# Funatiq/cuclark

Measured on AMD Instinct MI355X. Metric: Mreads/sec (10M x 150bp, k=31), higher is better.
Workload: dtype u64

## Files before the change

cuclark_amd/_lib.py:

```python
import ctypes as C
import importlib.util
import os
import subprocess

_PKG = os.path.dirname(os.path.abspath(__file__))
LIB_PATH = os.environ.get("MIC_LIB_PATH") or os.path.join(_PKG, "lib", "libmi_clark.so")
CSRC = os.path.join(_PKG, "csrc")

MIC_RESULT_WORDS = 8
MIC_FLAG_ROW_OVERFLOW = 1
MIC_FLAG_DENSE_PATH = 2
MIC_ROW_INVALID = 0xFFFFFFFF
MIC_ROLLUP_WORDS, MIC_ROLLUP_MAX_LEVELS = 8, 7
MIC_ROLLUP_UNRESOLVED, MIC_ROLLUP_PENDING = 0xFFFFFFFF, 0xFFFFFFFE
MIC_DENSITY_WORDS, MIC_DENSITY_CONF_BINS, MIC_DENSITY_GAMMA_BINS = 5153, 51, 101
MIC_KSKETCH_REGS = 16384
MIC_LAYOUT_AUTO, MIC_LAYOUT_DIRECT, MIC_LAYOUT_MINIMIZER, MIC_LAYOUT_SUPER, MIC_LAYOUT_SUPER2 = 0, 1, 2, 3, 4


class MicError(RuntimeError):
    def __init__(self, code, msg):
        super().__init__(f"libmi_clark error {code}: {msg}")
        self.code = code

# ... 44 lines not shown
    ("mic_db_load_host", C.c_int, [_VP, _VP, C.c_uint64, _VP, C.c_int, _VP, C.c_uint32, C.c_uint64, C.c_uint64]),
    ("mic_db_load_device", C.c_int, [_VP, _VP, C.c_uint64, _VP, C.c_int, _VP, C.c_uint32, C.c_uint64, C.c_uint64]),
    ("mic_db_set_part", C.c_int, [_VP, C.c_uint32, C.c_uint32]),
    ("mic_db_reserve_hbm", C.c_int, [_VP, C.c_uint64]),
    ("mic_peer_matrix", C.c_int, [C.POINTER(C.c_int), C.c_int]),
    ("mic_device_memory", C.c_int, [C.c_int, C.POINTER(C.c_uint64), C.POINTER(C.c_uint64)]),
    ("mic_db_load_files_multi", C.c_int, [C.POINTER(C.c_void_p), _SZ, C.c_char_p, C.c_int, C.c_uint32]),
    ("mic_db_kernel_name", C.c_int, [_VP, C.c_char_p, _SZ]),
    ("mic_db_get_info", C.c_int, [_VP, C.POINTER(MicDbInfo)]),
    ("mic_db_unload", C.c_int, [_VP]),
    ("mic_db_last_build_report", C.c_char_p, []),
    ("mic_batches_alloc", C.c_int, [_VP, _SZ, _SZ, _SZ, _U32P, C.c_int, C.POINTER(_VP), C.POINTER(_VP), C.POINTER(_VP),
                                    C.POINTER(_VP)]),
    ("mic_batch_ready", C.c_int, [_VP, _SZ, _SZ, _SZ]),
    ("mic_batch_query", C.c_int, [_VP, _SZ, C.c_int, C.c_int]),
    ("mic_batch_wait", C.c_int, [_VP, _SZ]),
    ("mic_batch_dense_counts", C.c_int, [_VP, _SZ, _SZ, _VP]),
    ("mic_batch_check", C.c_int, [_VP, _SZ, C.POINTER(C.c_int)]),
    ("mic_batch_merge_shards", C.c_int, [C.POINTER(C.c_void_p), _SZ, _SZ]),
    ("mic_batch_query_group", C.c_int, [C.POINTER(C.c_void_p), _SZ, _SZ, C.c_int]),
    ("mic_sync", C.c_int, [_VP]),
    ("mic_thread_bind_near_device", C.c_int, [_VP, C.c_int]),
    ("mic_batches_free", C.c_int, [_VP]),
    ("mic_query_device", C.c_int, [_VP, _VP, _VP, _SZ, _VP, _VP, _VP]),
    ("mic_resolve_flagged_device", C.c_int, [_VP, _VP, _VP, _VP, _VP, _VP, C.POINTER(_SZ)]),
    ("mic_merge_rows_device", C.c_int, [_VP, _VP, _VP, _VP, _SZ, _VP]),
    ("mic_result_from_rows_device", C.c_int, [_VP, _VP, _VP, _SZ, _VP]),
    ("mic_count_dense_device", C.c_int, [_VP, _VP, _VP, _VP, _SZ, _VP, _VP]),
    ("mic_result_from_dense_device", C.c_int, [_VP, _VP, _VP, _SZ, _VP, _VP, _VP]),
    ("mic_probe_stats_device", C.c_int, [_VP, _VP, _VP, _SZ, C.POINTER(C.c_uint64)]),
    ("mic_last_query_ms", C.c_int, [_VP, C.POINTER(C.c_float)]),
    ("mic_last_crowd_stats", C.c_int, [_VP, C.POINTER(C.c_uint32)]),
    ("mic_debug_fetch_crowd", C.c_int, [_VP, _VP, _SZ, C.POINTER(C.c_uint32)]),
    ("mic_debug_stream_pool", C.c_int, [C.POINTER(C.c_uint32)]),
    ("mic_ingest_alloc", C.c_int, [_VP, _SZ, _SZ, C.POINTER(C.c_char_p), C.c_uint32, C.c_int, C.POINTER(_VP)]),
    ("mic_ingest_classify", C.c_int, [_VP, _SZ, _SZ, C.c_int, C.POINTER(MicIngestResult)]),
    ("mic_ingest_classify_group", C.c_int, [C.POINTER(C.c_void_p), _SZ, _SZ, _SZ, _SZ, C.c_int, C.POINTER(MicIngestResult)]),
    ("mic_ingest_fetch_group_rows", C.c_int, [_VP, _SZ, _SZ, _VP, _SZ, C.POINTER(C.c_uint64), C.POINTER(C.c_uint32)]),
    ("mic_ingest_group_stats", C.c_int, [_VP, C.POINTER(C.c_double), _SZ]),
    ("mic_ingest_fetch_packed", C.c_int, [_VP, _SZ, _VP, _SZ, _VP, _SZ, C.POINTER(C.c_uint64), C.POINTER(C.c_uint64)]),
    ("mic_ingest_free", C.c_int, [_VP]),
    ("mic_ingest_set_min_quality", C.c_int, [_VP, C.c_uint32]),
    ("mic_fastq_mask_quality", C.c_int, [_VP, _SZ, C.c_uint32, _VP]),
    ("mic_ingest_set_low_complexity", C.c_int, [_VP, C.c_uint32]),
    ("mic_text_mask_low_complexity", C.c_int, [_VP, _SZ, C.c_uint32, _VP]),
    ("mic_gz_inflate_device", C.c_int, [_VP, _VP, _SZ, C.POINTER(_VP), C.POINTER(_SZ), C.POINTER(C.c_uint32)]),
    ("mic_gz_copy_text", C.c_int, [_VP, _VP, _SZ, _SZ, _VP]),
    ("mic_gz_free_text", C.c_int, [_VP, _VP]),
    ("mic_gz_reserve", C.c_int, [_VP, _SZ, C.c_uint32]),
    ("mic_gz_reserve_bytes", C.c_uint64, [_SZ, C.c_uint32]),
    ("mic_gz_release", C.c_int, [_VP]),
    ("mic_pairs_index_device", C.c_int, [_VP, _VP, _SZ, _VP, _SZ, C.POINTER(_VP), C.POINTER(C.c_uint64), C.POINTER(C.c_uint32)]),
    ("mic_pairs_offsets", C.c_int, [_VP, C.POINTER(C.POINTER(C.c_uint64)), C.POINTER(_SZ), C.POINTER(C.c_uint32)]),
    ("mic_pairs_merge_to_slot", C.c_int, [_VP, _VP, C.c_uint64, C.c_uint64, _SZ, C.POINTER(_SZ)]),
    ("mic_pairs_text", C.c_int, [_VP, _VP, C.c_uint64, C.c_uint64, _VP, _SZ, C.POINTER(_SZ)]),
    ("mic_pairs_free", C.c_int, [_VP, _VP]),
    ("mic_text_index_device", C.c_int, [_VP, _VP, _SZ, C.POINTER(_VP), C.POINTER(C.c_uint64), C.POINTER(C.c_uint32)]),
    ("mic_text_index_front_device", C.c_int, [_VP, _VP, _SZ, C.POINTER(_VP), C.POINTER(C.c_uint64), C.POINTER(C.c_uint64), C.POINTER(C.c_uint32)]),
    ("mic_gz_stream_open", C.c_int, [_VP, _VP, _SZ, C.c_uint32, C.POINTER(_VP), C.POINTER(_VP), C.POINTER(_SZ)]),
    ("mic_gz_stream_next", C.c_int, [_VP, C.POINTER(_SZ), C.POINTER(C.c_int)]),
    ("mic_gz_stream_close", C.c_int, [_VP, C.c_int]),
    ("mic_text_offsets", C.c_int, [_VP, C.POINTER(C.POINTER(C.c_uint64)), C.POINTER(_SZ), C.POINTER(C.c_uint32)]),
    ("mic_text_to_slot", C.c_int, [_VP, _VP, C.c_uint64, C.c_uint64, _SZ, C.POINTER(_SZ)]),
    ("mic_text_copy", C.c_int, [_VP, _VP, C.c_uint64, C.c_uint64, _VP, _SZ, C.POINTER(_SZ)]),
    ("mic_text_free", C.c_int, [_VP, _VP]),
    ("mic_text_format", C.c_int, [_VP]),
# ... 119 lines not shown
```

cuclark_amd/csrc/mic_engine.hip:

```cpp
#include "mi_clark.h"
#include "mic_internal.h"

#include <errno.h>
#include <stdarg.h>
#include <stdio.h>
#include <stdlib.h>
#include <string.h>
#include <time.h>

#include <sched.h>

#include <algorithm>
#include <mutex>
#include <string>
#include <atomic>
#include <thread>
#include <unistd.h>
#include <utility>
#include <vector>

static thread_local char g_err[512] = "";
thread_local uint64_t mic_build_reserved_hbm = 0;

namespace {
// ... 623 lines not shown
  if (e->d_flagged) hipFree(e->d_flagged);
  if (e->d_crowd) hipFree(e->d_crowd);
  if (e->abund.d_counts) hipFree(e->abund.d_counts);
  if (e->rollup.d_counts) hipFree(e->rollup.d_counts);
  if (e->density.d_counts) hipFree(e->density.d_counts);
  if (e->ksketch.d_regs) hipFree(e->ksketch.d_regs);
  if (e->rollup.d_block) hipFree(e->rollup.d_block);
  if (e->ev0) mic_event_put(e->ev0);
  if (e->ev1) mic_event_put(e->ev1);
  if (e->stream) mic_stream_put(e->stream);
  if (e->up_stream) mic_stream_put(e->up_stream);
  if (e->down_stream) mic_stream_put(e->down_stream);
  delete e;
  return MIC_OK;
}

int mic_db_unload(mic_engine* e) {
  if (!e) return mic_set_error(MIC_E_INVALID, "null engine");
  int rc = set_device(e);
  if (rc) return rc;
  hipDeviceSynchronize();
  if (e->slots) hipFree(e->slots);
  if (e->side) hipFree(e->side);
  if (e->d_sizes) hipFree(e->d_sizes);
  e->slots = nullptr; e->side = nullptr; e->d_sizes = nullptr; e->db_loaded = false;
  memset(&e->info, 0, sizeof(e->info));
  return MIC_OK;
}

int mic_db_get_info(const mic_engine* e, mic_db_info* info) {
  if (!e || !info) return mic_set_error(MIC_E_INVALID, "null argument");
  if (!e->db_loaded) return mic_set_error(MIC_E_STATE, "no database loaded");
  *info = e->info;
  return MIC_OK;
}

const char* mic_db_last_build_report(void) {
  static thread_local std::string copy;
  std::lock_guard<std::mutex> lk(g_report_mu);
  copy = g_report;
  return copy.c_str();
}

int mic_db_reserve_hbm(mic_engine* e, uint64_t bytes) {
  if (!e) return mic_set_error(MIC_E_INVALID, "null engine");
  e->reserve_hbm = bytes;
  return MIC_OK;
}

int mic_db_set_part(mic_engine* e, uint32_t part, uint32_t n_parts) {
  if (!e) return mic_set_error(MIC_E_INVALID, "null engine");
  if (n_parts > 1 && part >= n_parts) return mic_set_error(MIC_E_INVALID, "part %u of %u", part, n_parts);
  if (n_parts > 65536) return mic_set_error(MIC_E_INVALID, "too many parts");
  if (e->db_loaded) return mic_set_error(MIC_E_STATE, "set the part before the database is loaded");
  e->part = n_parts > 1 ? part : 0; e->n_parts = n_parts > 1 ? n_parts : 0;
  return MIC_OK;
}

int mic_db_load_device(mic_engine* e, const uint8_t* d_sizes, uint64_t htsize, const void* d_keys, int key_bytes,
                       const uint16_t* d_labels, uint32_t sampling, uint64_t s0, uint64_t s1) {
  if (!e || !d_sizes || !d_keys || !d_labels) return mic_set_error(MIC_E_INVALID, "null argument");
  if (key_bytes != 2 && key_bytes != 4 && key_bytes != 8) return mic_set_error(MIC_E_INVALID, "key_bytes must be 2, 4 or 8");
  int rc = set_device(e);
  if (rc) return rc;
  if ((rc = check_shard(htsize, s0, s1))) return rc;
  if ((rc = apply_part(e, htsize, s0, s1))) return rc;
// ... 726 lines not shown
```

cuclark_amd/csrc/mic_kernels.hip:

```cpp
#include "mic_internal.h"
#include "mic_device.h"
#include "mic_ksketch.h"
#include "mic_hitmap.h"
#include "mic_join2.h"

#include <stdlib.h>
#include <type_traits>

#ifndef MIC_EXP
#define MIC_EXP 0
#endif
#ifndef MIC_FUNNEL64
#define MIC_FUNNEL64 1
#endif
#ifndef MIC_X
#define MIC_X 0
#endif

namespace {

__device__ __forceinline__ uint4 load_slot_quarter(const uint4* p) {
  typedef unsigned int u4 __attribute__((ext_vector_type(4)));
  u4 t = __builtin_nontemporal_load((const u4*)p);
  return make_uint4(t.x, t.y, t.z, t.w);
}

__device__ __forceinline__ uint64_t kmer_from_dwords(uint32_t d0, uint32_t d1, uint32_t d2, int nt_in_dword, int k) {
  const int s = 2 * nt_in_dword;
  uint64_t a = ((uint64_t)d0 << 32) | d1;
#if MIC_FUNNEL64
  uint64_t x = (a << s) | ((uint64_t)d2 >> (32 - s));
#else
  uint64_t x = s ? ((a << s) | (uint64_t)(d2 >> (32 - s))) : a;
#endif
  return x >> (64 - 2 * k);
}


struct ReadAhead { uint32_t pp, pe, hdr, w; };

__device__ __forceinline__ void ahead_ptr(const MicQueryArgs& a, uint32_t r, ReadAhead& x) {
  if (r < a.n_reads) { x.pp = a.reads_ptr[r]; x.pe = a.reads_ptr[r + 1]; } else { x.pp = 0; x.pe = 0; }
}

__device__ __forceinline__ void ahead_window(const uint16_t* __restrict__ cont, uint32_t r, uint32_t n_reads, int lane,
                                             ReadAhead& x) {
  x.hdr = 0; x.w = 0;
  if (r < n_reads) {
    const uint32_t pp = __builtin_amdgcn_readfirstlane(x.pp);
// ... 135 lines not shown
  uint32_t vbl = acc.label1, vbc = acc.count;
  if (n_ent > 1) {
    bl = __builtin_amdgcn_readlane(acc.label1, 0); bc = __builtin_amdgcn_readlane(acc.count, 0);
    for (uint32_t i = 1; i < n_ent; ++i) {
      const uint32_t l1 = __builtin_amdgcn_readlane(acc.label1, i);
      const uint32_t c = __builtin_amdgcn_readlane(acc.count, i);
      const bool over_best = c > bc || (c == bc && l1 < bl);
      const bool over_second = c > sc || (c == sc && l1 < sl);
      if (over_best) { sc = bc; sl = bl; bc = c; bl = l1; }
      else if (over_second) { sc = c; sl = l1; }
    }
    vbl = bl; vbc = bc;
  }
  uint32_t flags = 0;
  if (a.rows) {
    uint32_t* row = a.rows + (size_t)r * a.row_words;
    bool fits = n_ent <= a.row_words - 1 && !overflow;
    uint32_t rank = 0;
    for (uint32_t i = 0; i < n_ent; ++i) {
      uint32_t li = __builtin_amdgcn_readlane(acc.label1, i);
      rank += li < acc.label1;
    }
    bool big = (uint32_t)lane < n_ent && acc.count > 0xFFFF;
    if (__ballot(big)) fits = false;
    if (fits) {
      if ((uint32_t)lane < n_ent) row[1 + rank] = (acc.count << 16) | (acc.label1 - 1);
      if (lane == 0) row[0] = n_ent;
    } else {
      if (lane == 0) row[0] = MIC_ROW_INVALID;
      flags |= MIC_FLAG_ROW_OVERFLOW_;
    }
  }
  if (overflow) flags |= MIC_FLAG_ROW_OVERFLOW_;
  if (lane == 0) {
    uint4 lo, hi;
    lo.x = total;
    lo.y = vbl;
    lo.z = vbc;
    lo.w = sl;
    hi.x = sc;
    hi.y = n_ent; hi.z = flags; hi.w = 0;
    uint4* out = (uint4*)(a.results + (size_t)r * 8);
    out[0] = lo; out[1] = hi;
  }
#if MIC_EXP & 2
  if (__builtin_expect(__builtin_amdgcn_readfirstlane(flags) != 0, 0)) if (a.flagged) {
#else
  if (__builtin_amdgcn_readfirstlane(flags) && a.flagged) {
#endif
    if (lane == 0) {
      uint32_t pos = atomicAdd(&a.flagged[0], 1u);
      if (pos < a.flagged_cap) a.flagged[1 + pos] = r;
    }
  }
}

template <bool KEY64>
__global__ void __launch_bounds__(256) query_kernel(const MicQueryArgs a) {
  const int lane = threadIdx.x & 63;
  const int j = lane & 3;
  const uint32_t wave0 = __builtin_amdgcn_readfirstlane(blockIdx.x * 4 + (threadIdx.x >> 6));
  const uint32_t n_waves = gridDim.x * 4;
  const MicTable& t = a.t;
  const int k = t.k;
  const uint4* __restrict__ slots = t.slots;
  const uint16_t* __restrict__ cont = a.cont;

// ... 729 lines not shown
              }
            }
          }
        };
        while (__ballot(sl0 != 0xFFFFFFFFu) | __ballot(sl1 != 0xFFFFFFFFu)) {
          uint32_t nx0, nx1;
          level(sl0, sl1, res0, res1, nx0, nx1);
          sl0 = nx0; sl1 = nx1;
        }
        tally2(res0, res1, acc, n_ent, overflow, total, lane);
      }
    }
    uint32_t t_hdr, t_pp, t_pe;
    asm volatile("s_waitcnt vmcnt(0)" ::: "memory");
    __builtin_amdgcn_wave_barrier();
    ahead_take(ahead_sel ? ahead1 : ahead0, n_pp, t_hdr, t_pp, t_pe);
    __builtin_amdgcn_wave_barrier();
    {
      uint64_t kp = (uint64_t)__builtin_amdgcn_kernarg_segment_ptr();
      asm volatile("" : "+s"(kp));
      const __attribute__((address_space(4))) MicQueryArgs* kc = (const __attribute__((address_space(4))) MicQueryArgs*)kp;
      struct { uint32_t* results; uint32_t* rows; uint32_t* flagged; uint32_t row_words, flagged_cap; } fa;
      fa.results = kc->results; fa.rows = kc->rows; fa.flagged = kc->flagged; fa.row_words = kc->row_words; fa.flagged_cap = kc->flagged_cap;
      finish_read(acc, n_ent, total, overflow, r, fa, lane);
    }
    ahead_issue(ahead_sel ? ahead0 : ahead1, t_pp, r + 3 * n_waves);
    ahead_sel ^= 1;
    cur_pp = n_pp; cur_pe = n_pe; cur_hdr = t_hdr; n_pp = t_pp; n_pe = t_pe;
  }
}


__device__ __forceinline__ uint64_t wballot(bool p) { return __builtin_amdgcn_ballot_w64(p); }

static_assert(MIC_RMAX <= 32, "tally_counts sums the first two rows of lanes");
#define MIC_R_CROWDED (-16)
__device__ __forceinline__ void tally_counts(uint32_t lab1, uint32_t cnt, RowAcc& acc, uint32_t& n_ent, uint32_t& overflow,
                                             uint32_t& total, int lane) {
  uint64_t mm = wballot(lab1 != 0);
  while (mm) {
    const uint32_t l1 = __builtin_amdgcn_readlane(lab1, __builtin_ctzll(mm));
    const bool mine = lab1 == l1;
    mm &= ~wballot(mine);
    const uint32_t c = mine ? cnt : 0u;
    uint32_t sum = 0;
    {
      uint32_t v = c;
      v += (uint32_t)__builtin_amdgcn_update_dpp(0, (int)v, 0x111, 0xF, 0xF, true);
      v += (uint32_t)__builtin_amdgcn_update_dpp(0, (int)v, 0x112, 0xF, 0xF, true);
      v += (uint32_t)__builtin_amdgcn_update_dpp(0, (int)v, 0x114, 0xF, 0xF, true);
      v += (uint32_t)__builtin_amdgcn_update_dpp(0, (int)v, 0x118, 0xF, 0xF, true);
      sum = __builtin_amdgcn_readlane(v, 15) + __builtin_amdgcn_readlane(v, 31);
    }
    total += sum;
    row_add(acc, n_ent, overflow, l1, sum, lane);
  }
}

template <int KK, int MM, bool FWD, bool PART>
__global__ void __launch_bounds__(64 * MIC_M_WPB, 32 / MIC_M_WPB) query_kernel_r(const MicQueryArgs a) {
  __shared__ uint4 s_stage[MIC_M_WPB][MIC_RMAX * MIC_MSTRIDE + (MIC_RMAX / 8 - 1) * MIC_R_SKEW];
  __shared__ uint16_t s_rec[MIC_M_WPB][132];
  __shared__ uint32_t s_ahead[MIC_M_WPB][2][64];
  __shared__ uint32_t s_part[PART ? MIC_M_WPB : 1][2];
  const int lane = threadIdx.x & 63;
  const int wv = __builtin_amdgcn_readfirstlane(threadIdx.x >> 6);
  uint4* stage = s_stage[wv];
  uint16_t* rec = s_rec[wv];
  const uint32_t wave0 = __builtin_amdgcn_readfirstlane(blockIdx.x * MIC_M_WPB + wv);
  const uint32_t n_waves = gridDim.x * MIC_M_WPB;
  const MicTable& t = a.t;
  if (PART) { if (lane == 0) { s_part[wv][0] = t.slot_lo; s_part[wv][1] = t.slot_cnt; } __builtin_amdgcn_wave_barrier(); }
  const int k = KK ? KK : t.k, m = MM ? MM : t.m, ctx = k - m;
  const uint4* __restrict__ slots = t.slots;
  const uint16_t* __restrict__ cont = a.cont;
  auto below = [](uint64_t mask) { return (uint32_t)__builtin_amdgcn_mbcnt_hi((uint32_t)(mask >> 32), __builtin_amdgcn_mbcnt_lo((uint32_t)mask, 0u)); };

  uint32_t* ahead0 = s_ahead[wv][0];
  uint32_t* ahead1 = s_ahead[wv][1];
  auto ahead_issue = [&](uint32_t* entry, uint32_t pp_w, uint32_t r_ptr) {
    const uint64_t abase = ((uint64_t)(cont + pp_w)) & ~3ULL;
    const uint32_t rr = r_ptr < a.n_reads ? r_ptr : a.n_reads - 1;
    const uint64_t pbase = (uint64_t)(a.reads_ptr + rr) - 48;
    int ln = lane;
    asm volatile("" : "+v"(ln));
    if (ln < 12)
      __builtin_amdgcn_global_load_lds((const __attribute__((address_space(1))) void*)((const uint32_t*)abase + lane),
                                       (__attribute__((address_space(3))) void*)entry, 4, 0, 0);
    uint64_t pb = pbase + 48;
    asm volatile("" : "+s"(pb));
    if (ln < 2)
      __builtin_amdgcn_global_load_lds((const __attribute__((address_space(1))) void*)((const uint32_t*)pb + lane),
                                       (__attribute__((address_space(3))) void*)(entry + 12), 4, 0, 0);
  };
  auto ahead_take = [&](const uint32_t* entry, uint32_t pp_w, uint32_t& hdr, uint32_t& npp, uint32_t& npe) {
    const uint32_t raw = entry[lane];
    npp = __builtin_amdgcn_readlane(raw, 12); npe = __builtin_amdgcn_readlane(raw, 13);
    const bool odd = (((uint64_t)(cont + pp_w)) >> 1) & 1;
    const uint32_t first = __builtin_amdgcn_readfirstlane(raw);
    hdr = odd ? first >> 16 : first & 0xFFFFu;
  };
  auto ahead_word = [&](const uint32_t* entry, uint32_t pp_w) {
    const uint32_t raw = entry[lane];
    const bool odd = (((uint64_t)(cont + pp_w)) >> 1) & 1;
    const uint32_t up = (uint32_t)__builtin_amdgcn_update_dpp(0, (int)raw, 0x101, 0xF, 0xF, true);
    return __builtin_amdgcn_perm(up, raw, odd ? 0x05040706u : 0x03020504u);
  };
  uint32_t cur_pp, cur_pe, cur_hdr, n_pp, n_pe, ahead_sel;
  {
    const uint32_t r0 = wave0 < a.n_reads ? wave0 : a.n_reads - 1;
    cur_pp = __builtin_amdgcn_readfirstlane(a.reads_ptr[r0]); cur_pe = __builtin_amdgcn_readfirstlane(a.reads_ptr[r0 + 1]);
    ahead_issue(ahead0, cur_pp, wave0 + n_waves);
    asm volatile("s_waitcnt vmcnt(0)" ::: "memory");
    __builtin_amdgcn_wave_barrier();
    ahead_take(ahead0, cur_pp, cur_hdr, n_pp, n_pe);
    ahead_issue(ahead1, n_pp, wave0 + 2 * n_waves);
    ahead_sel = 1;
  }
  constexpr bool PIPE = KK != 0 && (MIC_R_PIPE >= 2 || (MIC_R_PIPE == 1 && FWD));
  struct Round {
    uint32_t G0, G1, G2, cur;
    int jmax, jmin, remaining;
  };
  struct NoGap {};
  struct Gap { uint32_t len1, b2, g0; };
  auto front = [&](const uint32_t first, const uint32_t cend, const uint32_t base, const uint32_t nk, const bool use_ahead, uint32_t& wd_out,
                   const auto gp) __attribute__((always_inline)) -> uint32_t {
    constexpr bool GAP = std::is_same<decltype(gp), const Gap>::value;
    int ln = lane;
    asm volatile("" : "+v"(ln));
    uint32_t wd;
    if constexpr (GAP) {
      const uint32_t* entry = ahead_sel ? ahead0 : ahead1;
      const uint32_t j = (uint32_t)ln < 12u ? (uint32_t)ln : 0u;
      const uint32_t d = j2_dword(j, gp.len1, gp.b2);
      wd = j2_window(ahead_word(entry, cur_pp), entry[d], entry[d + 1u], j, gp.len1, gp.b2);
    } else {
      wd = use_ahead ? ahead_word(ahead_sel ? ahead0 : ahead1, cur_pp)
                     : window_word_w(cont, first, cend, base, ln, false, 0u);
    }
    wd_out = wd;
    const uint32_t n_act = nk - base < 128u ? nk - base : 128u;
    if constexpr (KK == F3_K && MM == F3_M) {
      uint32_t p0, s0, s1, s2, q0, q1, q2;
      if constexpr (GAP) sampled_positions3<!FWD, true>(wd, lane, n_act, p0, s0, s1, s2, q0, q1, q2, gp.len1, gp.g0);
      else sampled_positions3<!FWD>(wd, lane, n_act, p0, s0, s1, s2, q0, q1, q2);
      const uint32_t pv = (uint32_t)__builtin_amdgcn_update_dpp(-1, (int)q2, 0x138, 0xF, 0xF, false);
      const bool f0 = q0 != pv, f1 = q1 != q0, f2 = q2 != q1;
      const uint64_t b0 = wballot(f0), b1 = wballot(f1), b2 = wballot(f2);
// ... 66 lines not shown
    region_x(G0, G1, key, xhi);
    bool rev = false;
    if (!FWD) {
      const uint32_t sh = 96u - 2u * (uint32_t)(k + ctx);
      const uint32_t r0 = __builtin_bitreverse32(G2), r1 = __builtin_bitreverse32(G1), r2 = __builtin_bitreverse32(G0);
      uint32_t q0, q1, q2;
      if (KK != 0 && sh != 0) {
        q0 = swap_comp_pairs(__builtin_amdgcn_alignbit(r0, r1, 33u - sh), __builtin_amdgcn_alignbit(r0, r1, 31u - sh));
        q1 = swap_comp_pairs(__builtin_amdgcn_alignbit(r1, r2, 33u - sh), __builtin_amdgcn_alignbit(r1, r2, 31u - sh));
        q2 = swap_comp_pairs(r2 << (sh - 1u), r2 << (sh + 1u));
      } else {
        q0 = sh ? __builtin_amdgcn_alignbit(r0, r1, 32u - sh) : r0;
        q1 = sh ? __builtin_amdgcn_alignbit(r1, r2, 32u - sh) : r1;
        q2 = r2 << sh;
        q0 = swap_comp_pairs(q0 >> 1, q0 << 1); q1 = swap_comp_pairs(q1 >> 1, q1 << 1); q2 = swap_comp_pairs(q2 >> 1, q2 << 1);
      }
      uint32_t kr, hr;
      region_x(q0, q1, kr, hr);
      rev = hr < xhi || (hr == xhi && kr < key);
      G0 = rev ? q0 : G0; G1 = rev ? q1 : G1; G2 = rev ? q2 : G2;
      key = rev ? kr : key; xhi = rev ? hr : xhi;
    }
    const int jmaxf = qa - i0, jminf = jmaxf - n + 1;
    const int jmax = rev ? ctx - jminf : jmaxf, jmin = rev ? ctx - jmaxf : jminf;
    uint32_t cur = vr ? sslot_of_x32(key, xhi, (uint32_t)t.n_main) : 0xFFFFFFFFu;
    bool mine = vr;
    if (PART) {
      mine = vr && cur - s_part[wv][0] < s_part[wv][1];
      cur = mine ? cur : 0xFFFFFFFFu;
    }
    L.G0 = G0; L.G1 = G1; L.G2 = G2; L.cur = cur;
    L.jmax = jmax; L.jmin = jmin; L.remaining = mine ? n : 0;
  };
  auto issue = [&](const uint32_t cur, const uint32_t nrun) __attribute__((always_inline)) {
    uint32_t sidx[MIC_RMAX / 8];
    int ln = lane;
    asm volatile("" : "+v"(ln));
    __builtin_amdgcn_wave_barrier();
    if (ln < MIC_RMAX) ((uint32_t*)stage)[lane] = cur;
    __builtin_amdgcn_wave_barrier();
    uint32_t so = (uint32_t)(uintptr_t)(__attribute__((address_space(3))) void*)stage;
    asm volatile("" : "+s"(so));
#pragma unroll
    for (int i = 0; i < MIC_RMAX / 8; ++i) sidx[i] = ((const uint32_t*)stage)[8 * i + (lane >> 3)];
#pragma unroll
    for (int i = 0; i < MIC_RMAX / 8; ++i) {
      if (8u * i >= nrun) break;
      if (sidx[i] != 0xFFFFFFFFu)
        __builtin_amdgcn_global_load_lds((const __attribute__((address_space(1))) void*)(slots + (uint64_t)sidx[i] * 8 + (lane & 7)),
                                         (__attribute__((address_space(3))) void*)(uintptr_t)(so + 16u * (64 + MIC_R_SKEW) * (uint32_t)i), 16, 0, 0);
    }
  };
  auto consume = [&](Round& L, RowAcc& acc, uint32_t& n_ent, uint32_t& overflow, uint32_t& total, uint32_t& cg) __attribute__((always_inline)) {
    const uint32_t G0 = L.G0, G1 = L.G1, G2 = L.G2;
    uint32_t key, xhi_;
    region_x(G0, G1, key, xhi_);
    const int jmax = L.jmax, jmin = L.jmin;
    uint32_t cur = L.cur;
    int remaining = L.remaining;
    bool again = false;
    do {
      if (again) issue(cur, MIC_RMAX);
      again = true;
      asm volatile("s_waitcnt vmcnt(0)" ::: "memory");
      __builtin_amdgcn_wave_barrier();
      const bool vl = cur != 0xFFFFFFFFu;
      const uint32_t* q = (const uint32_t*)(stage + (vl ? staged_at((uint32_t)lane) : 0));
      const uint4 ka = *(const uint4*)q;
      const uint2 kb = *(const uint2*)(q + 4);
      uint32_t e = (ka.x < key) + (ka.y < key) + (ka.z < key) + (ka.w < key) + (kb.x < key) + (kb.y < key);
      const uint32_t mz = q[30];
      bool more = vl && e < 6;
      e = e < 5 ? e : 5;
      for (;;) {
        uint32_t e3 = e + (e << 1);
        asm volatile("" : "+v"(e3));
        uint32_t g = q[e], S0 = q[6 + e3], S1 = q[7 + e3], S2 = q[8 + e3], pl = q[24 + e];
        asm volatile("" : "+v"(S2));
        const bool same = more && g == key;
        const uint32_t d0 = G0 ^ S0, d1 = G1 ^ S1, d2 = G2 ^ S2;
        const bool mineq = k > 16
                               ? ((d0 & ((1u << ((32 - 2 * ctx) & 31)) - 1u)) | (d1 >> xsh)) == 0
                               : (((((uint64_t)d0 << 32) | d1) << (2 * ctx)) >> (64 - 2 * m)) == 0;
        const uint32_t dl = d0 >> (32 - 2 * ctx);
        const uint32_t dr = k > 16 ? __builtin_amdgcn_alignbit(d1, d2, xsh)
                                        : (uint32_t)((((((uint64_t)d0 << 32) | d1)) << ((2 * k) & 63)) >> 32);
        const int left = __builtin_ctz(dl | (1u << (2 * ctx))) >> 1;
        const int right = __builtin_clz(dr | (1u << (31 - 2 * ctx))) >> 1;
        const int hi = left < jmax ? left : jmax, lo = ctx - right > jmin ? ctx - right : jmin;
        const uint32_t range = ((2u << (hi & 31)) - 1u) & (~0u << (lo & 31));
        const uint32_t hits = (same && mineq) ? (uint32_t)__popc((pl >> 16) & range) : 0u;
#if !(MIC_X & 1)
        remaining = (same && mineq && (pl >> 16) == 0) ? MIC_R_CROWDED : remaining;
#endif
        const uint32_t lab_new = (pl & 0xFFFFu) + 1u;
        tally_counts(hits ? lab_new : 0u, hits, acc, n_ent, overflow, total, lane);
        remaining -= (int)hits;
        more = same && remaining > 0 && e < 5;
        e += more ? 1u : 0u;
        if (!wballot(more)) break;
      }
      const bool nx = vl && remaining > 0 && (mz & MIC_S_NEXT);
      cur = 0xFFFFFFFFu;
      if (wballot(nx)) { if (nx && q[5] <= key) cur = q[31]; }
    } while (wballot(cur != 0xFFFFFFFFu));
    if (!(MIC_X & 2) && __builtin_expect(wballot(remaining <= MIC_R_CROWDED) != 0, 0)) {
      const bool crowded = remaining <= MIC_R_CROWDED;
      const uint32_t n_c = (uint32_t)__popcll(wballot(crowded));
      uint64_t kpv = (uint64_t)__builtin_amdgcn_kernarg_segment_ptr();
      asm volatile("" : "+v"(kpv));
      const MicQueryArgs* kv = (const MicQueryArgs*)kpv;
      uint32_t* cw = kv->crowd;
      uint32_t* itb = kv->crowd_items;
      const uint32_t icap = kv->crowd_item_cap;
      uint32_t ib = 0xFFFFFFFFu;
      if (cw != nullptr && cg != MIC_CG_DENSE) {
        uint32_t v = 0;
        if (lane == 0) v = atomicAdd(&cw[1], n_c);
        ib = __builtin_amdgcn_readfirstlane(v);
      }
      asm volatile("" : "+v"(ib));
      const bool room = ib <= icap && n_c <= icap - ib;
      if (crowded && room) {
        uint32_t* it = itb + 8 * ((size_t)ib + below(wballot(crowded)));
        it[0] = G0; it[1] = G1; it[2] = G2; it[3] = (uint32_t)jmin | ((uint32_t)jmax << 8);
        it[4] = cg;
      }
      cg = __builtin_amdgcn_readfirstlane(room ? (ib | ((n_c - 1u) << 27)) : MIC_CG_DENSE);
    }
  };
  auto finish = [&](const RowAcc& acc, uint32_t n_ent, uint32_t total, uint32_t overflow, uint32_t r, const uint32_t cg) __attribute__((always_inline)) {
    uint32_t spilled = 0;
    if (!(MIC_X & 4) && __builtin_expect(cg != MIC_CG_NONE, 0)) {
      uint64_t kpv = (uint64_t)__builtin_amdgcn_kernarg_segment_ptr();
      asm volatile("" : "+v"(kpv));
      const MicQueryArgs* kv = (const MicQueryArgs*)kpv;
      uint32_t* cw = kv->crowd;
      uint32_t* pool = kv->crowd_pool;
// ... 48 lines not shown
      uint32_t n_wd = 0, R = MIC_RMAX + 1u, g0 = 0xFFFFFFFFu;
      if (PIPE && shape) {
        R = front(pp + 1, pp1, 0u, plen0 - (uint32_t)k + 1u, true, n_wd, NoGap{});
      } else if constexpr (PIPE) {
        const uint32_t odd = (uint32_t)((((uint64_t)(cont + cur_pp)) >> 1) & 1);
        const uint32_t* entry = ahead_sel ? ahead0 : ahead1;
        const J2Shape j2 = j2_shape(plen0, slot2, pe - pp, odd, (uint32_t)k,
                                    [&](uint32_t u) { return (uint32_t)__builtin_amdgcn_readfirstlane(j2_half(entry[u >> 1], u)); });
        if (__builtin_expect(j2.ok != 0u, 0)) {
          R = front(pp + 1, pp1, 0u, j2.n_act, true, n_wd, Gap{j2.len1, j2.b2, j2.g0});
          g0 = j2.g0;
        }
      }
      if (PIPE && R <= MIC_RMAX) { setup(n_wd, 0u, R, N, n_nrun, Gap{0u, 0u, g0}); simple = true; }
    }
    if (PIPE && p_valid) {
      RowAcc acc; acc.label1 = 0; acc.count = 0;
      uint32_t n_ent = 0, overflow = 0, total = 0, cg = MIC_CG_NONE;
      consume(P, acc, n_ent, overflow, total, cg);
      finish(acc, n_ent, total, overflow, r - n_waves, cg);
    } else {
      asm volatile("s_waitcnt vmcnt(0)" ::: "memory");
    }
    if (!have) return false;
    if (!simple) {
      RowAcc acc; acc.label1 = 0; acc.count = 0;
      uint32_t n_ent = 0, overflow = 0, total = 0, cg = MIC_CG_NONE;
      auto chunk = [&](const uint32_t first, const uint32_t cend, const uint32_t base, const uint32_t nk, const bool use_ahead) __attribute__((always_inline)) {
        uint32_t wd;
        const uint32_t R = front(first, cend, base, nk, use_ahead, wd, NoGap{});
        for (uint32_t rbase = 0; rbase < R; rbase += MIC_RMAX) {
          Round L; uint32_t nrun;
          setup(wd, rbase, R, L, nrun, NoGap{});
          issue(L.cur, nrun);
          consume(L, acc, n_ent, overflow, total, cg);
        }
      };
      if (!PIPE && shape) chunk(pp + 1, pp1, 0u, plen0 - (uint32_t)k + 1u, true);
      else {
        bool first_part = true;
        while (pp < pe) {
          uint32_t plen;
          {
            const uint32_t rel = pp - cur_pp + (uint32_t)((((uint64_t)(cont + cur_pp)) >> 1) & 1);
            if (first_part) plen = cur_hdr;
            else if (rel < 24u) {
              const uint32_t v = (ahead_sel ? ahead0 : ahead1)[rel >> 1];
              plen = __builtin_amdgcn_readfirstlane((rel & 1u) ? v >> 16 : v & 0xFFFFu);
            } else plen = __builtin_amdgcn_readfirstlane((uint32_t)cont[pp]);
          }
          const bool ahead_ok = first_part;
          first_part = false;
          if (plen == 0) break;
          const uint32_t first = pp + 1;
          pp = first + (plen + 7) / 8;
          if (plen < (uint32_t)k) continue;
          const uint32_t nk = plen - k + 1;
          const uint32_t cend = pp;
          for (uint32_t base = 0; base < nk; base += 128) chunk(first, cend, base, nk, ahead_ok && base == 0);
        }
      }
      finish(acc, n_ent, total, overflow, r, cg);
    }
    uint32_t t_hdr, t_pp, t_pe;
    __builtin_amdgcn_wave_barrier();
    ahead_take(ahead_sel ? ahead1 : ahead0, n_pp, t_hdr, t_pp, t_pe);
    __builtin_amdgcn_wave_barrier();
    ahead_issue(ahead_sel ? ahead0 : ahead1, t_pp, r + 3 * n_waves);
    ahead_sel ^= 1;
    cur_pp = n_pp; cur_pe = n_pe; cur_hdr = t_hdr; n_pp = t_pp; n_pe = t_pe;
    p_valid = simple;
    if (simple) issue(N.cur, n_nrun);
    r += n_waves;
    return true;
  };
  Round Ra, Rb;
  while (step(Ra, Rb) && step(Rb, Ra)) {}
}

__global__ void __launch_bounds__(256) crowd_finish_kernel(const MicQueryArgs a) {
  const int lane = threadIdx.x & 63;
  const uint32_t wave0 = __builtin_amdgcn_readfirstlane(blockIdx.x * 4 + (threadIdx.x >> 6)), n_waves = gridDim.x * 4;
  const uint32_t* __restrict__ cw = a.crowd;
  const uint32_t pcap = a.crowd_pend_cap;
  uint32_t np = cw[0];
  np = np < pcap ? np : pcap;
  const uint32_t* __restrict__ pend = cw + MIC_CROWD_HDR;
  const uint32_t* __restrict__ items = a.crowd_items;
  const uint32_t* __restrict__ pool = a.crowd_pool;
  const uint4* __restrict__ side = a.t.side;
  const uint32_t smask = a.t.side_mask;
  const int k = a.t.k, ctx = k - a.t.m;
  for (uint32_t p = wave0; p < np; p += n_waves) {
    const uint4 h = *(const uint4*)(pend + 8 * (size_t)p);
    const uint32_t r = __builtin_amdgcn_readfirstlane(h.x), meta = __builtin_amdgcn_readfirstlane(h.z), off = __builtin_amdgcn_readfirstlane(h.w);
    uint32_t total = __builtin_amdgcn_readfirstlane(h.y);
    uint32_t g = __builtin_amdgcn_readfirstlane(pend[8 * (size_t)p + 4]);
    if (meta == 0xFFFFFFFFu) continue;
    uint32_t n_ent = meta & 0xFFu, overflow = (meta >> 8) & 1u;
    RowAcc acc; acc.label1 = 0; acc.count = 0;
    if ((uint32_t)lane < n_ent) { const uint2 e = *(const uint2*)(pool + off + 2 * lane); acc.label1 = e.x; acc.count = e.y; }
    while (g != MIC_CG_NONE) {
      const uint32_t ib = g & 0x7FFFFFFu, n_c = (g >> 27) + 1u;
      g = __builtin_amdgcn_readfirstlane(items[8 * (size_t)ib + 4]);
      for (uint32_t b = 0; b < n_c; b += 4) {
// ... 577 lines not shown
```

cuclark_amd/db.py:

```python
import ctypes as C

import numpy as np

from . import _lib
from ._lib import MicConfig, MicDbInfo, MicError, check, MIC_RESULT_WORDS


class MiClarkUnsupported(RuntimeError):
    """mic_gz_*: an input the device path does not take (MIC_E_UNSUPPORTED); the caller uses its other path."""


def _as_np(ptr, shape, dtype):
    n = int(np.prod(shape))
    if n == 0:
        return np.zeros(shape, dtype)
    buf = (C.c_char * (n * np.dtype(dtype).itemsize)).from_address(ptr)
    return np.frombuffer(buf, dtype=dtype).reshape(shape)


class MiClarkDB:
    def __init__(self, k, num_targets, num_batches=1, device=-1, row_words=16, layout=0):
        self.L = _lib.load()
        self.k = int(k)
        self.num_targets = int(num_targets)
# ... 452 lines not shown
    def query_device(self, d_reads_pointer, d_containers, n_reads, d_results, d_rows=0, stream=0):
        check(self.L.mic_query_device(self.h, d_reads_pointer, d_containers, n_reads, d_results, d_rows or None,
                                      stream or None))

    def resolve_flagged_device(self, d_reads_pointer, d_containers, d_results, d_rows=0, stream=0):
        n = C.c_size_t(0)
        check(self.L.mic_resolve_flagged_device(self.h, d_reads_pointer, d_containers, d_results, d_rows or None,
                                                stream or None, C.byref(n)))
        return int(n.value)

    def merge_rows_device(self, d_a, d_b, d_out, n_reads, stream=0):
        check(self.L.mic_merge_rows_device(self.h, d_a, d_b, d_out, n_reads, stream or None))

    def result_from_rows_device(self, d_rows, d_results, n_reads, stream=0):
        check(self.L.mic_result_from_rows_device(self.h, d_rows, d_results, n_reads, stream or None))

    def count_dense_device(self, d_reads_pointer, d_containers, d_ids, n_ids, d_counts, stream=0):
        check(self.L.mic_count_dense_device(self.h, d_reads_pointer, d_containers, d_ids or None, n_ids, d_counts,
                                            stream or None))

    def result_from_dense_device(self, d_counts, d_ids, n_ids, d_results, d_rows=0, stream=0):
        check(self.L.mic_result_from_dense_device(self.h, d_counts, d_ids or None, n_ids, d_results, d_rows or None, stream or None))

    def probe_stats_device(self, d_reads_pointer, d_containers, n_reads):
        out = (C.c_uint64 * 4)()
        check(self.L.mic_probe_stats_device(self.h, d_reads_pointer, d_containers, n_reads, out))
        return dict(kmers=int(out[0]), probed=int(out[1]), hits=int(out[2]), bucket_len_sum=int(out[3]))

    def last_query_ms(self):
        ms = C.c_float(0)
        check(self.L.mic_last_query_ms(self.h, C.byref(ms)))
        return float(ms.value)

    def last_crowd_stats(self):
        out = (C.c_uint32 * 4)()
        check(self.L.mic_last_crowd_stats(self.h, out))
        return dict(reads=int(out[0]), runs=int(out[1]), row_words=int(out[2]), reads_to_dense_path=int(out[3]))
```

include/mi_clark.h:

```cpp
#ifndef MI_CLARK_H
#define MI_CLARK_H

#include <stddef.h>
#include <stdint.h>

#ifdef __cplusplus
extern "C" {
#endif

#define MIC_OK 0
#define MIC_E_INVALID (-1)
#define MIC_E_IO (-2)
#define MIC_E_NOMEM (-3)
#define MIC_E_HIP (-4)
#define MIC_E_STATE (-5)
#define MIC_E_NODEVICE (-6)
#define MIC_E_UNSUPPORTED (-7)

#define MIC_RESULT_WORDS 8
#define MIC_FLAG_ROW_OVERFLOW 1u
#define MIC_FLAG_DENSE_PATH 2u

#define MIC_ROW_INVALID 0xFFFFFFFFu
#define MIC_MAX_PART 65528u
// ... 64 lines not shown
const char* mic_db_last_build_report(void);

int mic_batches_alloc(mic_engine* e, size_t num_reads_total, size_t max_reads, size_t max_containers,
                      const uint32_t* index_batches, int extended, uint32_t** results, uint32_t** rows,
                      uint32_t** reads_pointer , uint16_t** containers );
int mic_batch_ready(mic_engine* e, size_t batch, size_t n_reads, size_t n_containers);
int mic_batch_query(mic_engine* e, size_t batch, int extended, int followup);
int mic_batch_wait(mic_engine* e, size_t batch);
int mic_batch_dense_counts(mic_engine* e, size_t batch, size_t read_in_batch, uint32_t* counts);
int mic_batch_check(mic_engine* e, size_t batch, int* done);
int mic_batch_merge_shards(mic_engine* const* engines, size_t n_engines, size_t batch);
int mic_batch_query_group(mic_engine* const* engines, size_t n_engines, size_t batch, int extended);
int mic_sync(mic_engine* e);
int mic_thread_bind_near_device(mic_engine* e, int on);
int mic_batches_free(mic_engine* e);

int mic_query_device(mic_engine* e, const uint32_t* d_reads_pointer, const uint16_t* d_containers, size_t n_reads,
                     uint32_t* d_results, uint32_t* d_rows, void* stream);
int mic_resolve_flagged_device(mic_engine* e, const uint32_t* d_reads_pointer, const uint16_t* d_containers,
                               uint32_t* d_results, uint32_t* d_rows, void* stream, size_t* n_resolved);
int mic_merge_rows_device(mic_engine* e, const uint32_t* d_rows_a, const uint32_t* d_rows_b, uint32_t* d_rows_out,
                          size_t n_reads, void* stream);
int mic_result_from_rows_device(mic_engine* e, const uint32_t* d_rows, uint32_t* d_results, size_t n_reads,
                                void* stream);
int mic_count_dense_device(mic_engine* e, const uint32_t* d_reads_pointer, const uint16_t* d_containers,
                           const uint32_t* d_read_ids, size_t n_ids, uint32_t* d_counts, void* stream);
int mic_result_from_dense_device(mic_engine* e, const uint32_t* d_counts, const uint32_t* d_ids, size_t n_ids,
                                 uint32_t* d_results, uint32_t* d_rows, void* stream);
int mic_probe_stats_device(mic_engine* e, const uint32_t* d_reads_pointer, const uint16_t* d_containers, size_t n_reads,
                           uint64_t out[4]);
int mic_last_query_ms(mic_engine* e, float* ms);
int mic_last_crowd_stats(mic_engine* e, uint32_t out[4]);
int mic_debug_fetch_crowd(mic_engine* e, uint32_t* out, size_t words, uint32_t caps[3]);

#define MIC_INGEST_PAIRED 1
#define MIC_INGEST_FASTQ_2LINE 2
#define MIC_INGEST_RESIDENT 4
#define MIC_INGEST_RESIDENT_FASTQ 12
#define MIC_INGEST_NO_CSV 16
#define MIC_INGEST_OK 0u
#define MIC_INGEST_FALLBACK 1u
#define MIC_INGEST_ODD_RECORD 2u
#define MIC_INGEST_TRUNCATED 4u
#define MIC_INGEST_LONG_READ 8u
#define MIC_INGEST_TOO_MANY 16u
#define MIC_INGEST_DENSE 32u

typedef struct mic_ingest_result {
  uint64_t n_reads;
  uint64_t csv_bytes;
  const char* csv;
  const uint32_t* results;
  uint32_t status;
  uint32_t n_lines;
} mic_ingest_result;

int mic_ingest_alloc(mic_engine* e, size_t n_slots, size_t max_bytes, const char* const* target_names, uint32_t n_targets,
                     int want_results, uint8_t** raw );
int mic_ingest_classify(mic_engine* e, size_t slot, size_t n_bytes, int flags, mic_ingest_result* out);
int mic_ingest_classify_group(mic_engine* const* group, size_t n_group, size_t owner, size_t slot, size_t n_bytes, int flags,
                              mic_ingest_result* out);
int mic_ingest_fetch_packed(mic_engine* e, size_t slot, uint32_t* reads_pointer, size_t rp_cap, uint16_t* containers,
                            size_t cont_cap, uint64_t* n_reads, uint64_t* n_containers);
int mic_ingest_fetch_group_rows(mic_engine* owner, size_t slot, size_t part, uint32_t* rows, size_t cap_words, uint64_t* n_reads,
                                uint32_t* row_words);
#define MIC_GROUP_STATS_FIELDS 10
// ... 166 lines not shown
```

Baseline: 2310.

## Stop bucket entry walk early via next-key ballot and wave-level masks

Rewrites the super-k-mer bucket probe loop to keep its control state as wave-wide ballot masks. It also peeks the next entry's key so the walk stops as soon as the following entry cannot match, rather than stepping through the rest. tally_counts now inserts new labels with writelane instead of calling row_add, and the issue of the next slot moves into the loop. Debug counters, a slot-fetch API and experiment switches guarded by MIC_X bits are added, which adds complexity and the risk of subtly changing which entries are counted.

```diff
diff --git a/cuclark_amd/_lib.py b/cuclark_amd/_lib.py
--- a/cuclark_amd/_lib.py
+++ b/cuclark_amd/_lib.py
@@ -100,6 +100,7 @@
     ("mic_last_query_ms", C.c_int, [_VP, C.POINTER(C.c_float)]),
     ("mic_last_crowd_stats", C.c_int, [_VP, C.POINTER(C.c_uint32)]),
     ("mic_debug_fetch_crowd", C.c_int, [_VP, _VP, _SZ, C.POINTER(C.c_uint32)]),
+    ("mic_debug_fetch_slots", C.c_int, [_VP, C.c_uint64, C.c_uint64, _VP]),
     ("mic_debug_stream_pool", C.c_int, [C.POINTER(C.c_uint32)]),
     ("mic_ingest_alloc", C.c_int, [_VP, _SZ, _SZ, C.POINTER(C.c_char_p), C.c_uint32, C.c_int, C.POINTER(_VP)]),
     ("mic_ingest_classify", C.c_int, [_VP, _SZ, _SZ, C.c_int, C.POINTER(MicIngestResult)]),
diff --git a/cuclark_amd/csrc/mic_engine.hip b/cuclark_amd/csrc/mic_engine.hip
--- a/cuclark_amd/csrc/mic_engine.hip
+++ b/cuclark_amd/csrc/mic_engine.hip
@@ -679,6 +679,19 @@
   if (!e || !info) return mic_set_error(MIC_E_INVALID, "null argument");
   if (!e->db_loaded) return mic_set_error(MIC_E_STATE, "no database loaded");
   *info = e->info;
+  return MIC_OK;
+}
+
+int mic_debug_fetch_slots(mic_engine* e, uint64_t first, uint64_t n, uint32_t* out) {
+  if (!e || !out) return mic_set_error(MIC_E_INVALID, "null argument");
+  if (!e->db_loaded) return mic_set_error(MIC_E_STATE, "no database loaded");
+  if (e->table.layout != 2 || e->table.parted) return mic_set_error(MIC_E_UNSUPPORTED, "slots are fetched from a whole super-k-mer table only");
+  if (first > e->info.n_slots || n > e->info.n_slots - first) return mic_set_error(MIC_E_INVALID, "slots [%llu, +%llu) of %llu",
+                                                                                   (unsigned long long)first, (unsigned long long)n, (unsigned long long)e->info.n_slots);
+  int rc = set_device(e);
+  if (rc) return rc;
+  MIC_TRY(hipDeviceSynchronize());
+  if (n) MIC_TRY(hipMemcpy(out, e->table.slots + first * 8, n * 128, hipMemcpyDeviceToHost));
   return MIC_OK;
 }
 
diff --git a/cuclark_amd/csrc/mic_kernels.hip b/cuclark_amd/csrc/mic_kernels.hip
--- a/cuclark_amd/csrc/mic_kernels.hip
+++ b/cuclark_amd/csrc/mic_kernels.hip
@@ -15,6 +15,15 @@
 #endif
 #ifndef MIC_X
 #define MIC_X 0
+#endif
+#if MIC_X & 8
+__device__ unsigned long long g_entry_walk[3];
+extern "C" int mic_debug_entry_walk(unsigned long long out[3], int reset) {
+  if (hipMemcpyFromSymbol(out, HIP_SYMBOL(g_entry_walk), sizeof(g_entry_walk)) != hipSuccess) return -1;
+  const unsigned long long z[3] = {0, 0, 0};
+  if (reset && hipMemcpyToSymbol(HIP_SYMBOL(g_entry_walk), z, sizeof(z)) != hipSuccess) return -1;
+  return 0;
+}
 #endif
 
 namespace {
@@ -216,7 +225,7 @@
     }
   }
   if (overflow) flags |= MIC_FLAG_ROW_OVERFLOW_;
-  if (lane == 0) {
+  if (lane == 0 && !(MIC_X & 128)) {
     uint4 lo, hi;
     lo.x = total;
     lo.y = vbl;
@@ -1012,6 +1021,11 @@
 
 
 __device__ __forceinline__ uint64_t wballot(bool p) { return __builtin_amdgcn_ballot_w64(p); }
+#if defined(__has_builtin) && __has_builtin(__builtin_amdgcn_writelane)
+__device__ __forceinline__ int mic_writelane(int value, int lane, int old) { return __builtin_amdgcn_writelane(value, lane, old); }
+#else
+extern "C" __device__ int mic_writelane(int value, int lane, int old) __asm("llvm.amdgcn.writelane.i32");
+#endif
 
 static_assert(MIC_RMAX <= 32, "tally_counts sums the first two rows of lanes");
 #define MIC_R_CROWDED (-16)
@@ -1033,7 +1047,15 @@
       sum = __builtin_amdgcn_readlane(v, 15) + __builtin_amdgcn_readlane(v, 31);
     }
     total += sum;
-    row_add(acc, n_ent, overflow, l1, sum, lane);
+    if (wballot(acc.label1 == l1)) {
+      if (acc.label1 == l1) acc.count += sum;
+    } else if (n_ent < 64) {
+      acc.label1 = (uint32_t)mic_writelane((int)l1, (int)n_ent, (int)acc.label1);
+      acc.count = (uint32_t)mic_writelane((int)sum, (int)n_ent, (int)acc.count);
+      ++n_ent;
+    } else {
+      overflow = 1;
+    }
   }
 }
 
@@ -1058,12 +1080,11 @@
 
   uint32_t* ahead0 = s_ahead[wv][0];
   uint32_t* ahead1 = s_ahead[wv][1];
-  auto ahead_issue = [&](uint32_t* entry, uint32_t pp_w, uint32_t r_ptr) {
+  auto lane_copy = [&]() { int ln = lane; asm volatile("" : "+v"(ln)); return ln; };
+  auto ahead_issue = [&](uint32_t* entry, uint32_t pp_w, uint32_t r_ptr, const int ln) {
     const uint64_t abase = ((uint64_t)(cont + pp_w)) & ~3ULL;
     const uint32_t rr = r_ptr < a.n_reads ? r_ptr : a.n_reads - 1;
     const uint64_t pbase = (uint64_t)(a.reads_ptr + rr) - 48;
-    int ln = lane;
-    asm volatile("" : "+v"(ln));
     if (ln < 12)
       __builtin_amdgcn_global_load_lds((const __attribute__((address_space(1))) void*)((const uint32_t*)abase + lane),
                                        (__attribute__((address_space(3))) void*)entry, 4, 0, 0);
@@ -1090,11 +1111,11 @@
   {
     const uint32_t r0 = wave0 < a.n_reads ? wave0 : a.n_reads - 1;
     cur_pp = __builtin_amdgcn_readfirstlane(a.reads_ptr[r0]); cur_pe = __builtin_amdgcn_readfirstlane(a.reads_ptr[r0 + 1]);
-    ahead_issue(ahead0, cur_pp, wave0 + n_waves);
+    ahead_issue(ahead0, cur_pp, wave0 + n_waves, lane_copy());
     asm volatile("s_waitcnt vmcnt(0)" ::: "memory");
     __builtin_amdgcn_wave_barrier();
     ahead_take(ahead0, cur_pp, cur_hdr, n_pp, n_pe);
-    ahead_issue(ahead1, n_pp, wave0 + 2 * n_waves);
+    ahead_issue(ahead1, n_pp, wave0 + 2 * n_waves, lane_copy());
     ahead_sel = 1;
   }
   constexpr bool PIPE = KK != 0 && (MIC_R_PIPE >= 2 || (MIC_R_PIPE == 1 && FWD));
@@ -1227,10 +1248,8 @@
     L.G0 = G0; L.G1 = G1; L.G2 = G2; L.cur = cur;
     L.jmax = jmax; L.jmin = jmin; L.remaining = mine ? n : 0;
   };
-  auto issue = [&](const uint32_t cur, const uint32_t nrun) __attribute__((always_inline)) {
+  auto issue = [&](const uint32_t cur, const uint32_t nrun, const int ln) __attribute__((always_inline)) {
     uint32_t sidx[MIC_RMAX / 8];
-    int ln = lane;
-    asm volatile("" : "+v"(ln));
     __builtin_amdgcn_wave_barrier();
     if (ln < MIC_RMAX) ((uint32_t*)stage)[lane] = cur;
     __builtin_amdgcn_wave_barrier();
@@ -1253,10 +1272,7 @@
     const int jmax = L.jmax, jmin = L.jmin;
     uint32_t cur = L.cur;
     int remaining = L.remaining;
-    bool again = false;
-    do {
-      if (again) issue(cur, MIC_RMAX);
-      again = true;
+    for (;;) {
       asm volatile("s_waitcnt vmcnt(0)" ::: "memory");
       __builtin_amdgcn_wave_barrier();
       const bool vl = cur != 0xFFFFFFFFu;
@@ -1265,18 +1281,23 @@
       const uint2 kb = *(const uint2*)(q + 4);
       uint32_t e = (ka.x < key) + (ka.y < key) + (ka.z < key) + (ka.w < key) + (kb.x < key) + (kb.y < key);
       const uint32_t mz = q[30];
-      bool more = vl && e < 6;
+      const uint64_t m_vl = wballot(vl);
+      uint64_t m_more = m_vl & wballot(e < 6), m_pos = 0;
       e = e < 5 ? e : 5;
+#if MIC_X & 8
+      uint32_t ew_pass = 0;
+#endif
       for (;;) {
         uint32_t e3 = e + (e << 1);
         asm volatile("" : "+v"(e3));
-        uint32_t g = q[e], S0 = q[6 + e3], S1 = q[7 + e3], S2 = q[8 + e3], pl = q[24 + e];
+        uint32_t g = q[e], g1 = q[e + 1], S0 = q[6 + e3], S1 = q[7 + e3], S2 = q[8 + e3], pl = q[24 + e];
         asm volatile("" : "+v"(S2));
-        const bool same = more && g == key;
+        const uint64_t m_same = m_more & wballot(g == key);
+        const uint64_t m_next = wballot(g1 == key);
         const uint32_t d0 = G0 ^ S0, d1 = G1 ^ S1, d2 = G2 ^ S2;
-        const bool mineq = k > 16
-                               ? ((d0 & ((1u << ((32 - 2 * ctx) & 31)) - 1u)) | (d1 >> xsh)) == 0
-                               : (((((uint64_t)d0 << 32) | d1) << (2 * ctx)) >> (64 - 2 * m)) == 0;
+        const uint64_t m_hit = m_same & (k > 16
+                                             ? wballot(((d0 & ((1u << ((32 - 2 * ctx) & 31)) - 1u)) | (d1 >> xsh)) == 0)
+                                             : wballot((((((uint64_t)d0 << 32) | d1) << (2 * ctx)) >> (64 - 2 * m)) == 0));
         const uint32_t dl = d0 >> (32 - 2 * ctx);
         const uint32_t dr = k > 16 ? __builtin_amdgcn_alignbit(d1, d2, xsh)
                                         : (uint32_t)((((((uint64_t)d0 << 32) | d1)) << ((2 * k) & 63)) >> 32);
@@ -1284,21 +1305,43 @@
         const int right = __builtin_clz(dr | (1u << (31 - 2 * ctx))) >> 1;
         const int hi = left < jmax ? left : jmax, lo = ctx - right > jmin ? ctx - right : jmin;
         const uint32_t range = ((2u << (hi & 31)) - 1u) & (~0u << (lo & 31));
-        const uint32_t hits = (same && mineq) ? (uint32_t)__popc((pl >> 16) & range) : 0u;
-#if !(MIC_X & 1)
-        remaining = (same && mineq && (pl >> 16) == 0) ? MIC_R_CROWDED : remaining;
+        const uint32_t hits = __builtin_amdgcn_inverse_ballot_w64(m_hit) ? (uint32_t)__popc((pl >> 16) & range) : 0u;
+#if MIC_X & 8
+        const bool ew_hit = wballot(hits != 0) != 0;
+        if (lane == 0 && ew_pass < 2u) atomicAdd(&g_entry_walk[ew_pass], 1ull);
+        if (lane == 0 && ew_pass == 1u && ew_hit) atomicAdd(&g_entry_walk[2], 1ull);
+        ++ew_pass;
 #endif
         const uint32_t lab_new = (pl & 0xFFFFu) + 1u;
+#if !(MIC_X & 16)
         tally_counts(hits ? lab_new : 0u, hits, acc, n_ent, overflow, total, lane);
+#endif
+#if MIC_X & 32
+        break;
+#endif
+#if !(MIC_X & 1)
+        remaining = __builtin_amdgcn_inverse_ballot_w64(m_hit & wballot(pl < 0x10000u)) ? MIC_R_CROWDED : remaining;
+#endif
         remaining -= (int)hits;
-        more = same && remaining > 0 && e < 5;
-        e += more ? 1u : 0u;
-        if (!wballot(more)) break;
+        m_pos = wballot(remaining > 0);
+        m_more = m_same & m_pos & wballot(e < 5);
+#if !(MIC_X & 256)
+        m_more &= m_next;
+#endif
+        e += __builtin_amdgcn_inverse_ballot_w64(m_more) ? 1u : 0u;
+        if (!m_more) break;
       }
-      const bool nx = vl && remaining > 0 && (mz & MIC_S_NEXT);
+#if MIC_X & 64
+      break;
+#endif
+      const uint64_t m_nx = m_pos & wballot((mz & MIC_S_NEXT) != 0);
+      if (!m_nx) break;
       cur = 0xFFFFFFFFu;
-      if (wballot(nx)) { if (nx && q[5] <= key) cur = q[31]; }
-    } while (wballot(cur != 0xFFFFFFFFu));
+      if (__builtin_amdgcn_inverse_ballot_w64(m_nx) && q[5] <= key) cur = q[31];
+      if (!wballot(cur != 0xFFFFFFFFu)) break;
+      remaining = (cur == 0xFFFFFFFFu && remaining > 0) ? 0 : remaining;
+      issue(cur, MIC_RMAX, lane_copy());
+    }
     if (!(MIC_X & 2) && __builtin_expect(wballot(remaining <= MIC_R_CROWDED) != 0, 0)) {
       const bool crowded = remaining <= MIC_R_CROWDED;
       const uint32_t n_c = (uint32_t)__popcll(wballot(crowded));
@@ -1413,7 +1456,7 @@
         for (uint32_t rbase = 0; rbase < R; rbase += MIC_RMAX) {
           Round L; uint32_t nrun;
           setup(wd, rbase, R, L, nrun, NoGap{});
-          issue(L.cur, nrun);
+          issue(L.cur, nrun, lane_copy());
           consume(L, acc, n_ent, overflow, total, cg);
         }
       };
@@ -1447,11 +1490,12 @@
     __builtin_amdgcn_wave_barrier();
     ahead_take(ahead_sel ? ahead1 : ahead0, n_pp, t_hdr, t_pp, t_pe);
     __builtin_amdgcn_wave_barrier();
-    ahead_issue(ahead_sel ? ahead0 : ahead1, t_pp, r + 3 * n_waves);
+    const int ln = lane_copy();
+    ahead_issue(ahead_sel ? ahead0 : ahead1, t_pp, r + 3 * n_waves, ln);
     ahead_sel ^= 1;
     cur_pp = n_pp; cur_pe = n_pe; cur_hdr = t_hdr; n_pp = t_pp; n_pe = t_pe;
     p_valid = simple;
-    if (simple) issue(N.cur, n_nrun);
+    if (simple) issue(N.cur, n_nrun, ln);
     r += n_waves;
     return true;
   };
diff --git a/cuclark_amd/db.py b/cuclark_amd/db.py
--- a/cuclark_amd/db.py
+++ b/cuclark_amd/db.py
@@ -508,6 +508,13 @@
         check(self.L.mic_last_query_ms(self.h, C.byref(ms)))
         return float(ms.value)
 
+    def fetch_slots(self, first=0, n=None):
+        if n is None:
+            n = int(self.info()["n_slots"]) - first
+        out = np.empty((n, 32), np.uint32)
+        check(self.L.mic_debug_fetch_slots(self.h, first, n, out.ctypes.data))
+        return out
+
     def last_crowd_stats(self):
         out = (C.c_uint32 * 4)()
         check(self.L.mic_last_crowd_stats(self.h, out))
diff --git a/include/mi_clark.h b/include/mi_clark.h
--- a/include/mi_clark.h
+++ b/include/mi_clark.h
@@ -120,6 +120,7 @@
 int mic_last_query_ms(mic_engine* e, float* ms);
 int mic_last_crowd_stats(mic_engine* e, uint32_t out[4]);
 int mic_debug_fetch_crowd(mic_engine* e, uint32_t* out, size_t words, uint32_t caps[3]);
+int mic_debug_fetch_slots(mic_engine* e, uint64_t first, uint64_t n, uint32_t* out);
 
 #define MIC_INGEST_PAIRED 1
 #define MIC_INGEST_FASTQ_2LINE 2
```

Result: faster. 2387, median of 6 (+3.3%).
